# Fadi987/PL-BERT

Measured on AMD Instinct MI355X. Metric: phoneme-tokens/sec, higher is better.
Workload: dtype bf16; 1 GPU; PL-BERT masked-phoneme training step (fwd+loss+bwd+allreduce+AdamW), ALBERT hidden 768 / 12 shared layers / FFN 2048 / 12 heads, seq_len 512, batch 32 per GPU; global_batch=32, seq_len=512, parallelism=dp1

## Files before the change

### plbert_amd/csrc/engine.cpp

```cpp
#include <dlfcn.h>
#include <hip/hip_runtime.h>
#include <math.h>
#include <stdarg.h>
#include <stdio.h>
#include <stdlib.h>
#include <string.h>

#include <array>
#include <map>
#include <new>
#include <string>

#include "../../include/plbert.h"
#include "plbert_kernels.h"

static thread_local char g_err[512] = "";
static int fail(const char* fmt, ...) {
  va_list ap;
  va_start(ap, fmt);
  vsnprintf(g_err, sizeof(g_err), fmt, ap);
  va_end(ap);
  return 1;
}
extern "C" const char* plb_last_error(void) { return g_err; }
// ... 126 lines not shown
  void access(int st, const void* p, size_t bytes, bool wr, const char* what) {
    if (!p || !bytes) return;
    const uintptr_t a = (uintptr_t)p, b = a + bytes;
    vc[st][st] += 1;
    for (const Acc& x : log) {
      if (x.st == st || !(wr || x.wr) || x.b <= a || b <= x.a) continue;
      ++checks;
      if (x.tick > vc[st][x.st]) {
        if (!violations++) {
          char m[384];
          snprintf(m, sizeof(m), "%s of '%s' on the %s stream is not ordered after the %s of '%s' on the %s stream", wr ? "write" : "read",
                   what, name(st), x.wr ? "write" : "read", x.what, name(x.st));
          first = m;
        }
      }
    }
    log.push_back(Acc{what, a, b, st, vc[st][st], wr});
  }
  void new_call() { log.clear(); waits = 0; }
};

}

struct PlbEngine {
  PlbConfig c;
  int64_t poff[PLB_NPARAM], psize[PLB_NPARAM], ptotal, ptrain;
  int E, H, I, L, NH, V, P, NP, NT;
  int64_t Tcap;
  int64_t NMcap;
  int64_t o_wbf, o_wqkvT, o_wdT, o_w1T, o_w2T, o_wpT, o_winT;
  int64_t o_e, o_x, o_qkv, o_ctx, o_pre1, o_a, o_u, o_g, o_pre2;
  int64_t o_lse, o_delta, o_mean1, o_rstd1, o_mean2, o_rstd2;
  int64_t o_dqkv, o_dpre1, o_du, o_dpre2;
  int64_t o_dy0, o_dy1, o_da, o_dctx, o_de;
  int64_t o_hm, o_logm, o_dlog, o_dhm, o_rows, o_tgt, o_w, o_lrows;
  int64_t o_slab, o_part1, o_part2, o_parte, o_scratch, o_dxe, o_ducol, o_slab2, o_scratch2, o_qkvcol = 0;
  int qkvcol_rows = 0;
  int64_t slab2_floats;
  int NTp = 0;
  int64_t o_bt = 0, o_wtT = 0, o_tdl = 0, o_tlrows = 0, o_tscr = 0, o_tgrad = 0, o_tloss = 0;
  int64_t o_tpmax = 0, o_tpsum = 0, o_ttl = 0, o_tlse = 0, o_tw = 0, o_ttgt = 0, o_tcolp = 0;
  bool tok_pad_zeroed = false;
  bool tok_grads_live = false;
  hipStream_t side = nullptr;
  hipEvent_t ev_fork = nullptr, ev_join = nullptr;
  int64_t slab_floats;
  int64_t ws_bytes;
  int ln_blocks, emb_blocks;
  int part_rows = 0;
  int part_rows_used = 0;
  int ln_fuse = 3;
  int64_t o_lnx = 0, o_lnerr = 0, lnx_bytes = 0;
  unsigned int* host_err = nullptr;
  unsigned int* host_err_dev = nullptr;
  bool gelu_dstash_on = true;
  bool u_is_derivative = false;
  bool fp8_on = false, fp8_ready = false, fp8_bwd_ready = false, fp8_wstale = true;
  bool fp8_tn = true;
  bool tn8_call = false;
  int64_t o_x8 = 0, o_a8 = 0, o_g8 = 0, o_c8 = 0, o_dp8 = 0, o_du8 = 0, o_dp18 = 0, o_dq8 = 0;
  int64_t o_wq8 = 0, o_wd8 = 0, o_w18 = 0, o_w28 = 0, o_w2T8 = 0, o_w1T8 = 0, o_wqT8 = 0, o_wdT8 = 0;
  int64_t o_f8amax = 0, o_f8scale = 0, o_f8deq = 0, o_f8stats = 0;
  int f8n = 0;
  bool infer = false;
  int pruned_rows = 0;
  int64_t last_app_rows[2] = {0, 0};
  int64_t last_exec_rows[2] = {0, 0};
// ... 127 lines not shown
  if (tr) {
    e->o_wqkvT = cv.take(rup(H, 128) * 3 * H * 2);
    e->o_wdT = cv.take(rup(H, 128) * H * 2);
    e->o_w1T = cv.take(rup(H, 128) * I * 2);
    e->o_w2T = cv.take(rup(I, 128) * H * 2);
    e->o_wpT = cv.take(rup(H, 128) * 256 * 2);
    e->o_winT = cv.take(rup(E, 128) * H * 2);
  }
  e->o_e = cv.take(Tp * E * 2);
  e->o_x = cv.take((tr ? L + 1 : 2) * Tp * H * 2);
  e->o_qkv = cv.take(Ls * Tp * 3 * H * 2);
  e->o_ctx = cv.take(Ls * Tp * H * 2);
  e->o_pre1 = cv.take(Ls * Tp * H * 2);
  e->o_a = cv.take(Ls * Tp * H * 2);
  e->o_u = cv.take(Ls * Tp * I * 2);
  e->o_g = cv.take(Ls * Tp * I * 2);
  e->o_pre2 = cv.take(Ls * Tp * H * 2);
  const int64_t stat = (int64_t)c.max_batch * e->NH * c.max_seq * 4;
  e->o_lse = cv.take(Ls * stat);
  e->o_mean1 = cv.take(Ls * Tp * 4); e->o_rstd1 = cv.take(Ls * Tp * 4);
  e->o_mean2 = cv.take(Ls * Tp * 4); e->o_rstd2 = cv.take(Ls * Tp * 4);
  e->lnx_bytes = (Tp / 128) * 16 * 128 * 2 * 8;
  e->o_lnx = cv.take(e->lnx_bytes);
  e->o_lnerr = cv.take(256);
  if (tr) {
    e->o_delta = cv.take(stat);
    e->o_dqkv = cv.take(L * Tp * 3 * H * 2);
    e->o_dpre1 = cv.take(L * Tp * H * 2);
    e->o_du = cv.take(L * Tp * I * 2);
    e->o_dpre2 = cv.take(L * Tp * H * 2);
    e->o_dy0 = cv.take(Tp * H * 2); e->o_dy1 = cv.take(Tp * H * 2);
    e->o_da = cv.take(Tp * H * 2); e->o_dctx = cv.take(Tp * H * 2);
    e->o_de = cv.take(Tp * E * 2);
  }
  const int64_t NM = e->NMcap;
  e->o_hm = cv.take(NM * H * 2);
  e->o_logm = cv.take(NM * 256 * 4);
  e->o_dlog = cv.take(NM * 256 * 2);
  e->o_rows = cv.take(NM * 4); e->o_tgt = cv.take(NM * 4); e->o_w = cv.take(NM * 4); e->o_lrows = cv.take(NM * 4);
  if (tr) {
    e->o_dhm = cv.take(NM * H * 2);
    int64_t slab = 0;
    {
      const int64_t Mtot = L * Tp;
      const int ntp = (int)rup(e->NT, 256);
      const int shapes[7][2] = {{(int)(3 * H), (int)H}, {(int)H, (int)H}, {(int)I, (int)H}, {(int)H, (int)I}, {(int)H, (int)E}, {e->NP, (int)H}, {ntp, (int)H}};
      for (int i = 0; i < (e->NT ? 7 : 6); ++i) {
        int rps;
        const int64_t mt = i < 4 ? Mtot : Tp;
        const int s = tn_splits(mt, shapes[i][0], shapes[i][1], &rps);
        const int64_t f = (int64_t)s * shapes[i][0] * shapes[i][1];
        if (f > slab) slab = f;
      }
    }
    e->slab_floats = slab;
    e->o_slab = cv.take(slab * 4);
    e->o_part1 = cv.take(L * e->part_rows * 3 * H * 4);
    e->o_part2 = cv.take(L * e->part_rows * 3 * H * 4);
    e->o_parte = cv.take((int64_t)e->emb_blocks * 2 * E * 4);
    e->o_dxe = cv.take(Tp * E * 4);
    e->o_ducol = cv.take(L * (2 * Tp / 128) * I * 4);
    e->qkvcol_rows = c.max_batch * ((c.max_seq + 127) / 128) * 4;
    e->o_qkvcol = cv.take((int64_t)L * e->qkvcol_rows * 3 * H * 4);
    e->o_scratch = cv.take(512 * (3 * H > I ? 3 * H : I) * 4);
    e->o_scratch2 = cv.take(512 * (3 * H > I ? 3 * H : I) * 4);
    {
// ... 418 lines not shown
}
static int gemm_ln_bwd(PlbEngine* e, PlbGemmNT* g, const F8Op* f8, bool fused, const LnSlot& ln, int nblocks, bf16_t* dx, int T,
                       int Tzero, uint8_t* dx8, const F8Site& q, hipStream_t s) {
  if (fused) {
    g->C = dx; g->aux = ln.pre; g->ldaux = e->H; g->colpart = ln.partials;
    ln_fields(e, g, ln.gamma, nullptr, ln.mean, ln.rstd);
    if (dx8) f8_out(g, dx8, e->H, q, 1);
    TRY(gemm_nt_ln_any(g, 6, f8, s));
    return 0;
  }
  TRY(gemm_nt_any(g, 0, f8, s));
  return ln_bwd(e, ln, nblocks, g->C, dx, T, Tzero, dx8, q, s);
}

static bool tn8_ok(const PlbEngine* e, int64_t Mtot);
static bool f8_call(const PlbEngine* e, int64_t Tp, bool train) {
  return e->fp8_on && e->fp8_ready && (!train || e->fp8_bwd_ready) && fp8_shapes_ok(e, Tp);
}
struct Prune { const int32_t* rows; int n; int Mc; };
static int g_prune_last = -1;
extern "C" void plb_set_prune_last(int on) { g_prune_last = on < 0 ? -1 : (on ? 1 : 0); }
static bool prune_enabled() {
  static const bool v = [] { const char* e = getenv("PLBERT_PRUNE_LAST"); return !(e && !strcmp(e, "0")); }();
  return g_prune_last < 0 ? v : g_prune_last != 0;
}
static int last_application_fwd_pruned(PlbEngine* e, const Prune* pr, bool stash, bool calib, bool tn8, const Slots& sl,
                                       const bf16_t* ctx_att, hipStream_t s) {
  const int H = e->H, I = e->I, L = e->L, Mc = pr->Mc, n = pr->n;
  const F8Site sA(e, F8_A, L - 1), sG(e, F8_G, L - 1), sC(e, F8_C, L - 1);
  bf16_t* ctxc = stash ? sl.ctx : sl.pre1;
  bf16_t* xc = stash ? e->at<bf16_t>(e->o_da) : sl.a;
  bf16_t* pre1c = stash ? sl.pre1 : sl.ctx;
  bf16_t* ac = stash ? sl.a : sl.pre1;
  TRY(plb_launch_gather_rows(ctx_att, H, pr->rows, n, Mc, H, ctxc, H, s));
  TRY(plb_launch_gather_rows(sl.x, H, pr->rows, n, Mc, H, xc, H, s));
  PlbGemmNT g = nt_desc(ctxc, e->wbf(PLB_DENSE_W), Mc, H, H);
  g.bias = e->par(PLB_DENSE_B); g.res = xc; g.ldr = H; g.C = pre1c; g.ldc = H;
  const LnSlot ln1 = {e->par(PLB_LN1_W), e->par(PLB_LN1_B), pre1c, sl.mean1, sl.rstd1, nullptr};
  if (gemm_ln_fwd(e, &g, nullptr, false, ln1, ac, Mc, nullptr, F8Site(), s)) return 1;
  if (calib) TRY(plb_launch_amax(ac, 1, (size_t)n, H, H, sA.amax, s));
  g = nt_desc(ac, e->wbf(PLB_FFN_W), Mc, I, H);
  g.bias = e->par(PLB_FFN_B); g.C = sl.u; g.ldc = I; g.C2 = sl.g; g.ldc2 = I;
  TRY(plb_launch_gemm_nt(&g, 1, 0, s));
  if (calib) TRY(plb_launch_amax(sl.g, 1, (size_t)n, I, I, sG.amax, s));
  g = nt_desc(sl.g, e->wbf(PLB_FFNO_W), Mc, H, I);
  g.bias = e->par(PLB_FFNO_B); g.res = ac; g.ldr = H; g.C = sl.pre2; g.ldc = H;
  if (gemm_ln_fwd(e, &g, nullptr, false, ln2_slot(e, sl), e->at<bf16_t>(e->o_hm), Mc, nullptr, F8Site(), s)) return 1;
  if (tn8) {
    const void* src[3] = {ctxc, ac, sl.g}; const int fl[3] = {1, 1, 1};
    const size_t nel[3] = {(size_t)Mc * H, (size_t)Mc * H, (size_t)Mc * I};
    const float* sc[3] = {sC.scale, sA.scale, sG.scale};
    uint8_t* dst[3] = {sl.c8, sl.a8, sl.g8};
    float* am[3] = {sC.amax, sA.amax, sG.amax};
    TRY(plb_launch_quantize_multi(3, src, fl, nel, sc, dst, am, s));
  }
  return 0;
}

static int run_encoder(PlbEngine* e, const int64_t* ids, const int32_t* lengths, int B, int S, const Rows& rw, bool stash,
                       bf16_t** xout, hipStream_t s, const Prune* pr = nullptr) {
  const int E = e->E, H = e->H, I = e->I, L = e->L;
  const int T = rw.T;
  const int64_t Tp = rw.Tp;
  const bool f8 = f8_call(e, Tp, stash);
  const bool calib = e->fp8_on && !f8;
  if (e->fp8_on && e->fp8_wstale) TRY(fp8_quantize_weights(e, s));
  PlbEmbed em;
  memset(&em, 0, sizeof(em));
// ... 439 lines not shown

static int last_application_bwd_pruned(PlbEngine* e, const Bwd& c, const Slots& sl, const Prune* pr) {
  const int H = e->H, I = e->I, L = e->L, Mc = pr->Mc, n = pr->n;
  hipStream_t s = c.s;
  const F8Site sDP(e, F8_DP, L - 1), sDU(e, F8_DU, L - 1), sDP1(e, F8_DP1, L - 1);
  bf16_t* const dac = e->at<bf16_t>(e->o_da);
  bf16_t* const dctxc = e->at<bf16_t>(e->o_dy0);
  bf16_t* const dctx = e->at<bf16_t>(e->o_dctx);
  if (ln_bwd(e, ln2_slot(e, sl), c.prows, e->at<bf16_t>(e->o_dhm), sl.dpre2, Mc, Mc, nullptr, F8Site(), s)) return 1;
  if (c.calib) TRY(plb_launch_amax(sl.dpre2, 1, (size_t)n, H, H, sDP.amax, s));
  PlbGemmNT g = nt_desc(sl.dpre2, e->at<bf16_t>(e->o_w2T), Mc, I, H);
  g.aux = sl.u; g.ldaux = I; g.C = sl.du; g.ldc = I;
  TRY(plb_launch_gemm_nt(&g, 2, 0, s));
  if (c.calib) TRY(plb_launch_amax(sl.du, 1, (size_t)n, I, I, sDU.amax, s));
  if (c.du_rows > 0) {
    TRY(plb_launch_colsum(sl.du, 1, (size_t)Mc, I, I, sl.ducol, I, 0, e->at<float>(e->o_scratch), 16, s));
    if (c.du_rows > 1) HIPTRY(hipMemsetAsync(sl.ducol + I, 0, (size_t)(c.du_rows - 1) * I * 4, s));
  }
  g = nt_desc(sl.du, e->at<bf16_t>(e->o_w1T), Mc, H, I);
  g.res = sl.dpre2; g.ldr = H; g.C = dac; g.ldc = H;
  if (gemm_ln_bwd(e, &g, nullptr, false, ln1_slot(e, sl), c.prows, sl.dpre1, Mc, Mc, nullptr, F8Site(), s)) return 1;
  if (c.calib) TRY(plb_launch_amax(sl.dpre1, 1, (size_t)n, H, H, sDP1.amax, s));
  if (e->tn8_call) {
    const void* src[3] = {sl.dpre2, sl.du, sl.dpre1}; const int fl[3] = {3, 3, 3};
    const size_t nel[3] = {(size_t)Mc * H, (size_t)Mc * I, (size_t)Mc * H};
    const float* sc[3] = {sDP.scale, sDU.scale, sDP1.scale};
    uint8_t* dst[3] = {sl.dp8, sl.du8, sl.dp18};
    float* am[3] = {sDP.amax, sDU.amax, sDP1.amax};
    TRY(plb_launch_quantize_multi(3, src, fl, nel, sc, dst, am, s));
  }
  g = nt_desc(sl.dpre1, e->at<bf16_t>(e->o_wdT), Mc, H, H);
  g.C = dctxc; g.ldc = H;
  TRY(plb_launch_gemm_nt(&g, 0, 0, s));
  HIPTRY(hipMemsetAsync(dctx, 0, (size_t)c.Tp * H * 2, s));
  TRY(plb_launch_scatter_rows(dctxc, H, pr->rows, n, H, dctx, H, s));
  HIPTRY(hipMemsetAsync(dac, 0, (size_t)c.Tp * H * 2, s));
  TRY(plb_launch_scatter_rows(sl.dpre1, H, pr->rows, n, H, dac, H, s));
  return 0;
}

static int attention_bwd_dx(PlbEngine* e, const Bwd& c, int l, const Slots& sl, bf16_t* ctx, const bf16_t* res,
                            bf16_t* dx) {
  const int H = e->H, T = c.T;
  hipStream_t s = c.s;
  const F8Site sDQ(e, F8_DQ, l);
  PlbAttn at;
  memset(&at, 0, sizeof(at));
  at.qkv = sl.qkv; at.ldqkv = 3 * H; at.lengths = c.lengths; at.B = c.B; at.S = c.S; at.NH = e->NH; at.H = H; at.scale = 0.125f;
  at.row_start = c.row_start;
  at.ctx = ctx; at.ldctx = H; at.lse = sl.lse;
  at.dctx = e->at<bf16_t>(e->o_dctx); at.lddctx = H; at.delta = e->at<float>(e->o_delta); at.dqkv = sl.dqkv; at.lddqkv = 3 * H;
  at.colpart = sl.qkvcol; at.colpart_accumulate = 0;
  if (c.f8) {
    at.dqkv8 = sl.dq8; at.lddqkv8 = 3 * H; at.dqkv_scale = sDQ.scale; at.dqkv_amax = sDQ.amax;
    if (e->tn8_call) at.dqkv = nullptr;
  }
  TRY(plb_launch_attn_bwd(&at, s));
  if (c.Tp > T) {
    if (at.dqkv) HIPTRY(hipMemsetAsync(sl.dqkv + (int64_t)T * 3 * H, 0, (size_t)(c.Tp - T) * 3 * H * 2, s));
    if (c.f8) HIPTRY(hipMemsetAsync(sl.dq8 + (int64_t)T * 3 * H, 0, (size_t)(c.Tp - T) * 3 * H, s));
  }
  if (c.calib) TRY(plb_launch_amax(sl.dqkv, 1, (size_t)T, 3 * H, 3 * H, sDQ.amax, s));
  PlbGemmNT g = nt_desc(sl.dqkv, e->at<bf16_t>(e->o_wqkvT), c.Tp, H, 3 * H);
  g.res = res; g.ldr = H; g.C = dx; g.ldc = H;
  const F8Op ox = f8_op(sl.dq8, sDQ, F8Weight(e, F8W_QKVT), 1);
  if (l == 0) {
    TRY(gemm_nt_any(&g, 0, c.f8 ? &ox : nullptr, s));
    return 0;
  }
  const Slots below = slots(e, c.Tp, c.B, c.S, l - 1, true, c.prows, c.du_rows);
// ... 537 lines not shown
```

### plbert_amd/csrc/gemm.hip

```cpp
#include "common.h"
#include "plbert_kernels.h"
#include "gemm_epilogue.h"

namespace {

constexpr int BM = 128, BN = 128, BK = 64;

DEVI int nt_lds_off(int row, int chunk) { return row * BK + ((chunk ^ ((row >> 1) & 7)) << 3); }

template <int ACT, bool OUTF32>
__global__ __launch_bounds__(256) void gemm_nt_kernel(PlbGemmNT p) {
  __shared__ __attribute__((aligned(16))) bf16_t smem[2][2][BM * BK];
  const int tid = threadIdx.x, lane = tid & 63, wave = tid >> 6;
  const int wr = wave >> 1, wc = wave & 1;
  const int nbn = (p.N + BN - 1) / BN;
  const int nwg = gridDim.x;
  const int logical = xcd_remap(blockIdx.x, nwg);
  const int bm = logical / nbn, bn = logical % nbn;

  const int uw = __builtin_amdgcn_readfirstlane(wave);
  const int drow = lane >> 3, dch = lane & 7;
  const bf16_t* gA = p.A + (size_t)(bm * BM + uw * 32 + drow) * p.lda;
  const bf16_t* gB = p.B + (size_t)(bn * BN + uw * 32 + drow) * p.ldb;
  const size_t sa = (size_t)8 * p.lda, sb = (size_t)8 * p.ldb;
  int sch[4];
#pragma unroll
  for (int i = 0; i < 4; ++i) sch[i] = (dch ^ ((4 * i + (lane >> 4)) & 7)) * 8;
  typedef __attribute__((address_space(1))) const void* gptr_t;
  typedef __attribute__((address_space(3))) void* lptr_t;
#define NT_STAGE(st, kt)                                                                              \
  do {                                                                                                \
    _Pragma("unroll") for (int i = 0; i < 4; ++i) {                                                   \
      __builtin_amdgcn_global_load_lds((gptr_t)(gA + i * sa + (size_t)(kt) * BK + sch[i]),            \
                                       (lptr_t)&smem[st][0][(uw * 32 + i * 8) * BK], 16, 0, 0);       \
      __builtin_amdgcn_global_load_lds((gptr_t)(gB + i * sb + (size_t)(kt) * BK + sch[i]),            \
                                       (lptr_t)&smem[st][1][(uw * 32 + i * 8) * BK], 16, 0, 0);       \
    }                                                                                                 \
  } while (0)
#define NT_LANDED() asm volatile("s_waitcnt vmcnt(0)" ::: "memory")

  f32x4 acc[4][4];
#pragma unroll
  for (int i = 0; i < 4; ++i)
#pragma unroll
    for (int j = 0; j < 4; ++j) acc[i][j] = f32x4{0.f, 0.f, 0.f, 0.f};

  const int frow = lane & 15, fq = lane >> 4;
  const int fsw = (frow >> 1) & 7;
  const int offA = (wr * 64 + frow) * BK, offB = (wc * 64 + frow) * BK;
#define NT_COMPUTE(st)                                                                                   \
  do {                                                                                                   \
    const bf16_t* sA = smem[st][0];                                                                      \
    const bf16_t* sB = smem[st][1];                                                                      \
    _Pragma("unroll") for (int kk = 0; kk < 2; ++kk) {                                                   \
      const int ch = ((kk * 4 + fq) ^ fsw) << 3;                                                         \
      bf16x8 af[4], bfr[4];                                                                              \
      _Pragma("unroll") for (int i = 0; i < 4; ++i) {                                                    \
        af[i] = *(const bf16x8*)&sA[offA + i * 16 * BK + ch];                                            \
        bfr[i] = *(const bf16x8*)&sB[offB + i * 16 * BK + ch];                                           \
      }                                                                                                  \
      _Pragma("unroll") for (int mi = 0; mi < 4; ++mi)                                                   \
        _Pragma("unroll") for (int ni = 0; ni < 4; ++ni)                                                 \
          acc[mi][ni] = __builtin_amdgcn_mfma_f32_16x16x32_bf16(bfr[ni], af[mi], acc[mi][ni], 0, 0, 0);  \
    }                                                                                                    \
  } while (0)

  const int nk = p.K / BK;
  NT_STAGE(0, 0);
  NT_LANDED();
  __syncthreads();
  for (int kt = 0; kt < nk; ++kt) {
    const int cur = kt & 1;
    if (kt + 1 < nk) NT_STAGE(cur ^ 1, kt + 1);
    NT_COMPUTE(cur);
    NT_LANDED();
    __syncthreads();
  }
#undef NT_STAGE
#undef NT_LANDED
#undef NT_COMPUTE

#pragma unroll
  for (int mi = 0; mi < 4; ++mi) {
    const int m = bm * BM + wr * 64 + mi * 16 + frow;
#pragma unroll
    for (int ni = 0; ni < 4; ++ni)
      nt_epilogue<ACT, OUTF32>(p, acc[mi][ni], m, bn * BN + wc * 64 + ni * 16 + fq * 4);
  }
}

DEVI int tn_unit(int t) { return (t & 3) | (((t >> 3) & 1) << 2) | (((t >> 2) & 1) << 3) | (t & 48); }
DEVI int tn_lds_off(int t, int col) {
  int s = col >> 4;
  return s * 1024 + (((tn_unit(t) + s) & 63) << 4) + (col & 15);
}

__global__ __launch_bounds__(256) void gemm_tn_kernel(PlbGemmTN p) {
  __shared__ __attribute__((aligned(16))) bf16_t smem[2][2][64 * 128];
  const int tid = threadIdx.x, lane = tid & 63, wave = tid >> 6;
  const int wn = wave >> 1, wk = wave & 1;
  const int nbk = (p.K + 127) / 128;
  const int bn = blockIdx.x / nbk, bk = blockIdx.x % nbk;
  const int split = blockIdx.y;
  const int t_begin = split * p.rows_per_split;
  int t_end = t_begin + p.rows_per_split;
  if (t_end > p.Mtot) t_end = p.Mtot;
  const int nt = (t_end - t_begin) / 64;

  const int lc = tid & 15, lr = tid >> 4;
  const int colA = bn * 128 + lc * 8, colB = bk * 128 + lc * 8;
  const bool okA = colA < p.Ncols, okB = colB < p.K;
  uint4 ra[4], rb[4];
  auto load_tile = [&](int it) {
    const size_t t0 = (size_t)t_begin + (size_t)it * 64 + lr;
#pragma unroll
    for (int i = 0; i < 4; ++i) {
      ra[i] = okA ? *(const uint4*)(p.A + (t0 + 16 * i) * p.lda + colA) : make_uint4(0, 0, 0, 0);
      rb[i] = okB ? *(const uint4*)(p.B + (t0 + 16 * i) * p.ldb + colB) : make_uint4(0, 0, 0, 0);
    }
  };
// ... 38 lines not shown
        bfr[i] = bf16x8{b0[0], b0[1], b0[2], b0[3], b1[0], b1[1], b1[2], b1[3]};
      }
#pragma unroll
      for (int ni = 0; ni < 4; ++ni)
#pragma unroll
        for (int ki = 0; ki < 4; ++ki)
          acc[ni][ki] = __builtin_amdgcn_mfma_f32_16x16x32_bf16(bfr[ki], af[ni], acc[ni][ki], 0, 0, 0);
    }
    if (it + 1 < nt) store_tile(cur ^ 1);
    __syncthreads();
  }

  float* out = p.slab + (size_t)split * p.N * p.K;
#pragma unroll
  for (int ni = 0; ni < 4; ++ni) {
    const int n = bn * 128 + wn * 64 + ni * 16 + li;
    if (n >= p.N) continue;
#pragma unroll
    for (int ki = 0; ki < 4; ++ki) {
      const int k0 = bk * 128 + wk * 64 + ki * 16 + 4 * g;
      if (k0 >= p.K) continue;
      f32x4 v = acc[ni][ki];
      *(float4*)(out + (size_t)n * p.K + k0) = make_float4(v[0], v[1], v[2], v[3]);
    }
  }
}

}

static int g_nt_tile = 0;
extern "C" void plb_set_gemm_nt_tile(int tile) { g_nt_tile = tile; }
extern "C" int plb_launch_gemm_nt_big(const PlbGemmNT* p, int tile, int act, int out_f32, hipStream_t stream);

static int pick_tile(const PlbGemmNT* p) {
  const bool ok256 = p->M % 256 == 0 && p->N % 256 == 0, ok384 = p->M % 128 == 0 && p->N % 384 == 0;
  const bool ok1256 = p->M % 128 == 0 && p->N % 256 == 0;
  if (g_nt_tile == 128) return 128;
  if (g_nt_tile == 256) return ok256 ? 256 : 128;
  if (g_nt_tile == 384) return ok384 ? 384 : (ok256 ? 256 : 128);
  if (g_nt_tile == 1256) return ok1256 ? 1256 : 128;
  if ((long)p->M * p->N < 256L * 256 * 64) return 128;
  double e256 = 0, e384 = 0, e1256 = 0;
  if (ok256) { const long t = (long)(p->M / 256) * (p->N / 256); e256 = (double)t / (double)(((t + 255) / 256) * 256); }
  if (ok384) { const long t = (long)(p->M / 128) * (p->N / 384); e384 = 0.95 * (double)t / (double)(((t + 255) / 256) * 256); }
  if (ok1256) { const long t = (long)(p->M / 128) * (p->N / 256); e1256 = 0.85 * (double)t / (double)(((t + 255) / 256) * 256); }
  if (e256 == 0 && e384 == 0 && e1256 == 0) return 128;
  if (e1256 > e256 && e1256 > e384) return 1256;
  return e384 > e256 ? 384 : 256;
}

extern "C" int plb_gemm_nt_colpart_rows(int M, int N, int K) {
  PlbGemmNT q;
  q.M = M; q.N = N; q.K = K;
  const int tile = pick_tile(&q);
  return tile == 256 ? 2 * (M / 256) : (tile == 384 || tile == 1256) ? 2 * (M / 128) : 0;
}

extern "C" int plb_launch_gemm_nt(const PlbGemmNT* p, int act, int out_f32, hipStream_t stream) {
  if (p->M % BM || p->K % BK || p->N % 4 || p->M <= 0 || p->N <= 0 || p->K <= 0) return 1;
  const int nbn = (p->N + BN - 1) / BN;
  dim3 grid((p->M / BM) * nbn), block(256);
  const int cls = out_f32 ? PLB_K_GEMM_NT_F32 : act == 1 ? PLB_K_GEMM_NT_GELU : act == 2 ? PLB_K_GEMM_NT_GELUBWD : PLB_K_GEMM_NT;
  const int tile = pick_tile(p);
  if (p->colpart && tile == 128) return 1;
  const double mnk = (double)p->M * p->N * p->K;
  const double algo_bytes = 2.0 * ((double)p->M * p->K + (double)p->N * p->K) +
                            (double)p->M * p->N * (out_f32 ? 4 : act == 1 ? 4 : 2) +
                            (p->res ? 2.0 * p->M * p->N : 0.0) + (act == 2 ? 2.0 * p->M * p->N : 0.0);
  if (tile != 128) {
    const int tokb = plb_prof_begin(cls, stream, 2.0 * mnk, algo_bytes);
    const int rc = plb_launch_gemm_nt_big(p, tile, act, out_f32, stream);
    plb_prof_end(tokb, stream);
    return rc;
  }
  const int tok = plb_prof_begin(out_f32 ? PLB_K_GEMM_NT_F32 : PLB_K_GEMM_NT_SMALL, stream, 2.0 * mnk, algo_bytes);
  if (out_f32) {
    if (act != 0) return 1;
    hipLaunchKernelGGL((gemm_nt_kernel<0, true>), grid, block, 0, stream, *p);
  } else if (act == 0) {
    hipLaunchKernelGGL((gemm_nt_kernel<0, false>), grid, block, 0, stream, *p);
  } else if (act == 1) {
    hipLaunchKernelGGL((gemm_nt_kernel<1, false>), grid, block, 0, stream, *p);
  } else if (act == 2) {
    hipLaunchKernelGGL((gemm_nt_kernel<2, false>), grid, block, 0, stream, *p);
  } else {
    return 1;
  }
  plb_prof_end(tok, stream);
  return hipGetLastError() == hipSuccess ? 0 : 2;
}

extern "C" int plb_launch_gemm_tn(const PlbGemmTN* p, hipStream_t stream) {
  if (p->Mtot % 64 || p->rows_per_split % 64 || p->K % 4 || p->N <= 0 || p->splits <= 0) return 1;
  if ((long)p->splits * p->rows_per_split < p->Mtot) return 1;
  dim3 grid(((p->N + 127) / 128) * ((p->K + 127) / 128), p->splits), block(256);
  const int tok = plb_prof_begin(PLB_K_GEMM_TN, stream, 2.0 * p->Mtot * (double)p->N * p->K,
                                 2.0 * p->Mtot * ((double)p->N + p->K) + 4.0 * p->splits * (double)p->N * p->K);
  hipLaunchKernelGGL(gemm_tn_kernel, grid, block, 0, stream, *p);
  plb_prof_end(tok, stream);
  return hipGetLastError() == hipSuccess ? 0 : 2;
}
```

### plbert_amd/csrc/plbert_kernels.h

```cpp
#pragma once
#include <hip/hip_runtime.h>
#include <stdint.h>

typedef uint16_t bf16_t;

extern "C" {

enum PlbKernelClass {
  PLB_K_GEMM_NT = 0, PLB_K_GEMM_NT_GELU, PLB_K_GEMM_NT_GELUBWD, PLB_K_GEMM_NT_F32, PLB_K_GEMM_TN,
  PLB_K_ATTN_FWD, PLB_K_ATTN_BWD_DQ, PLB_K_ATTN_BWD_DKV, PLB_K_LN_FWD, PLB_K_LN_BWD, PLB_K_EMBED_FWD,
  PLB_K_EMBED_BWD, PLB_K_COLSUM, PLB_K_REDUCE, PLB_K_ROWS, PLB_K_CE, PLB_K_ADAMW, PLB_K_CAST, PLB_K_TOKEN_CE, PLB_K_GEMM_NT_CE, PLB_K_GEMM_NT_SMALL, PLB_K_FP8, PLB_K_ATTN_BWD,
  PLB_K_GEMM_NT_FP8, PLB_K_GEMM_NT_GELU_FP8, PLB_K_GEMM_NT_GELUBWD_FP8,
  PLB_K_GEMM_NT_LNFWD, PLB_K_GEMM_NT_LNBWD,
  PLB_K_GEMM_NT_LNFWD_FP8, PLB_K_GEMM_NT_LNBWD_FP8, PLB_K_GEMM_TN_FP8,
  PLB_K_NCLASS
};
int plb_prof_begin(int cls, hipStream_t s, double flops, double bytes);
void plb_prof_end(int tok, hipStream_t s);

typedef struct {
  const bf16_t* A; int lda;
  const bf16_t* B; int ldb;
  int M, N, K;
  int Mstore;
// ... 94 lines not shown
int plb_launch_copy_cols(const float* scratch, int nsplit, int N, int col0, int Nout, float* out, hipStream_t stream);

int plb_launch_pooler(const float* hidden, int B, int S, int H, const float* W, const float* bias, float* pooled,
                      hipStream_t stream);

typedef struct {
  const bf16_t* qkv; int ldqkv;
  const int32_t* lengths;
  int B, S, NH, H;
  float scale;
  bf16_t* ctx; int ldctx;
  float* lse;
  const bf16_t* dctx; int lddctx;
  float* delta;
  bf16_t* dqkv; int lddqkv;
  float* colpart;
  int colpart_accumulate;
  uint8_t* ctx8; int ldctx8; const float* ctx_scale; float* ctx_amax;
  uint8_t* dqkv8; int lddqkv8; const float* dqkv_scale; float* dqkv_amax;
  const int32_t* qoff; const bf16_t* q; int ldq; int nq_total; bf16_t* dq; int lddq; uint8_t* dq8; int lddq8;
  const int32_t* row_start;
} PlbAttn;
int plb_launch_attn_fwd(const PlbAttn* p, hipStream_t stream);
int plb_launch_attn_bwd(const PlbAttn* p, hipStream_t stream);
int plb_launch_attn_bwd_fused(const PlbAttn* p, hipStream_t stream);
void plb_debug_skip_piece(int index);
void plb_debug_ln_fault(int mode, int launches);
void plb_set_attn_bwd_fused(int on);

int plb_launch_gather_rows(const bf16_t* src, int lds_, const int32_t* rows, int n, int npad, int H, bf16_t* dst,
                           int ldd, hipStream_t stream);
int plb_launch_scatter_rows(const bf16_t* src, int lds_, const int32_t* rows, int n, int H, bf16_t* dst, int ldd,
                            hipStream_t stream);
int plb_launch_ce_prepare(const int32_t* offsets, const int32_t* flat, const int64_t* labels, int B, int S,
                          int32_t* rows, int32_t* tgt, float* w, hipStream_t stream);
int plb_launch_ce_prepare_packed(const int32_t* offsets, const int32_t* flat, const int64_t* labels, int B, int S,
                                 const int32_t* row_start, int32_t* rows, int32_t* tgt, float* w, hipStream_t stream);
int plb_launch_unpack_rows(const void* src, int src_is_bf16, int lds_, const int32_t* row_start, const int32_t* lengths,
                           int B, int S, int C, float* dst, hipStream_t stream);
int plb_launch_ce_fwd_bwd(const float* logits, int ldl, int V, const int32_t* tgt, const float* w, int n, int npad,
                          float* loss_rows, bf16_t* dlogits, int ldd, hipStream_t stream);
int plb_launch_sum_rows(const float* x, int n, float* out, hipStream_t stream);
int plb_launch_token_ce_combine(const float* pmax, const float* psum, int ntiles, const float* tlogit,
                                const int32_t* lengths, int B, int S, int rows, float* lse, float* w, float* loss_rows,
                                hipStream_t stream);
int plb_launch_add_scalar(float* out, const float* a, const float* b, hipStream_t stream);

typedef struct {
  const int64_t* labels; const int32_t* lengths;
  int B, S;
  uint64_t seed; uint32_t step;
  float word_pred_prob, mask_prob, replace_prob;
  int mask_id, sep_id;
  int64_t* masked; int32_t *counts, *idx_padded, *offsets, *flat;
} PlbMask;
int plb_launch_mask(const PlbMask* p, hipStream_t stream);

typedef struct {
  const int64_t* ids; const int32_t *sample_off, *word_off, *word_begin, *word_len; const int8_t* action;
  const int64_t* repl; const int64_t* word_token; int64_t sep_token; const int32_t* crop_start;
  int B, S, mask_id;
  int64_t *labels, *masked, *tokens; int32_t *lengths_out, *counts, *idx_padded, *offsets, *flat;
} PlbApplyMask;
int plb_launch_apply_mask(const PlbApplyMask* p, hipStream_t stream);

int plb_launch_adamw(float* p, const float* g, float* m, float* v, bf16_t* p_bf16, size_t n, double lr, double beta1,
// ... 12 lines not shown
```

### plbert_amd/csrc/rowops.hip

```cpp
#include "common.h"
#include "plbert_kernels.h"

namespace {

__device__ __forceinline__ bool packed_locate(const int32_t* row_start, const int32_t* lengths, int B, int S, int r, int* b_out,
                                              int* s_out) {
  int lo = 0, hi = B;
  while (hi - lo > 1) {
    const int mid = (lo + hi) >> 1;
    if (row_start[mid] <= r) lo = mid; else hi = mid;
  }
  int len = lengths[lo];
  len = len < 1 ? 1 : (len > S ? S : len);
  *b_out = lo; *s_out = r - row_start[lo];
  return *s_out < len;
}

template <bool BWD>
__global__ __launch_bounds__(256) void embed_kernel(PlbEmbed p) {
  const int lane = threadIdx.x & 63, wave = threadIdx.x >> 6;
  const int E = p.E;
  const int c = lane * 4;
  const bool act = c < E;
  float4 g4 = make_float4(0, 0, 0, 0), b4 = g4, ty = g4;
// ... 665 lines not shown
    int k = g;
    for (; k + 24 < nsplit; k += 32) {
      s0 += px[(size_t)k * N]; s1 += px[(size_t)(k + 8) * N]; s2 += px[(size_t)(k + 16) * N]; s3 += px[(size_t)(k + 24) * N];
    }
    for (; k < nsplit; k += 8) s0 += px[(size_t)k * N];
  }
  red[g][c] = (s0 + s1) + (s2 + s3);
  __syncthreads();
  if (g == 0 && j < Nout) {
    const float t = ((red[0][c] + red[1][c]) + (red[2][c] + red[3][c])) + ((red[4][c] + red[5][c]) + (red[6][c] + red[7][c]));
    out[j] = accumulate ? out[j] + t : t;
  }
}

__global__ void gather_rows_kernel(const bf16_t* src, int lds_, const int32_t* rows, int n, int npad, int H,
                                   bf16_t* dst, int ldd) {
  const int r = blockIdx.x;
  const int chunks = H / 8;
  const bool live = r < n;
  const size_t srow = live ? (size_t)rows[r] : 0;
  for (int c = threadIdx.x; c < chunks; c += blockDim.x) {
    uint4 v = live ? *(const uint4*)(src + srow * lds_ + c * 8) : make_uint4(0, 0, 0, 0);
    *(uint4*)(dst + (size_t)r * ldd + c * 8) = v;
  }
}
__global__ void scatter_rows_kernel(const bf16_t* src, int lds_, const int32_t* rows, int n, int H, bf16_t* dst,
                                    int ldd) {
  const int r = blockIdx.x;
  if (r >= n) return;
  const size_t drow = (size_t)rows[r];
  for (int c = threadIdx.x; c < H / 8; c += blockDim.x)
    *(uint4*)(dst + drow * ldd + c * 8) = *(const uint4*)(src + (size_t)r * lds_ + c * 8);
}
__global__ void ce_prepare_kernel(const int32_t* offsets, const int32_t* flat, const int64_t* labels, int B, int S,
                                  const int32_t* row_start, int32_t* rows, int32_t* tgt, float* w) {
  __shared__ int cnt[4];
  int c = 0;
  for (int b = threadIdx.x; b < B; b += blockDim.x) c += offsets[b + 1] > offsets[b];
  c = (int)wave_sum((float)c);
  if ((threadIdx.x & 63) == 0) cnt[threadIdx.x >> 6] = c;
  __syncthreads();
  const int count = cnt[0] + cnt[1] + cnt[2] + cnt[3];
  const int b = blockIdx.x;
  const int j0 = offsets[b], j1 = offsets[b + 1];
  const float wb = (j1 > j0) ? 1.0f / ((float)(j1 - j0) * (float)count) : 0.f;
  for (int j = j0 + threadIdx.x; j < j1; j += blockDim.x) {
    const int idx = flat[j];
    rows[j] = row_start ? row_start[b] + idx : b * S + idx;
    tgt[j] = (int32_t)labels[(size_t)b * S + idx];
    w[j] = wb;
  }
}
template <typename T>
__global__ __launch_bounds__(256) void unpack_rows_kernel(const T* src, int lds_, const int32_t* row_start, const int32_t* lengths,
                                                          int S, int C, float* dst) {
  const int b = blockIdx.x / S, s = blockIdx.x - b * S;
  int len = lengths[b];
  len = len < 1 ? 1 : (len > S ? S : len);
  float* d = dst + (size_t)blockIdx.x * C;
  if (s >= len) {
    for (int c = threadIdx.x; c < C; c += 256) d[c] = 0.f;
    return;
  }
  const T* r = src + (size_t)(row_start[b] + s) * lds_;
  for (int c = threadIdx.x; c < C; c += 256) {
    if constexpr (sizeof(T) == 2) d[c] = bf2f(r[c]); else d[c] = r[c];
// ... 370 lines not shown
                                 int accumulate, float* scratch, int nsplit, hipStream_t stream) {
  if (N % 8 || ld % 8 || nsplit <= 0 || Nout > N) return 1;
  ProfScope ps(PLB_K_COLSUM, stream, 0, (double)R * N * (is_bf16 ? 2 : 4));
  dim3 grid((N + 255) / 256, nsplit);
  if (is_bf16) hipLaunchKernelGGL((colsum_kernel<true>), grid, dim3(256), 0, stream, X, R, N, ld, scratch, nsplit);
  else hipLaunchKernelGGL((colsum_kernel<false>), grid, dim3(256), 0, stream, X, R, N, ld, scratch, nsplit);
  if (hipGetLastError() != hipSuccess) return 2;
  hipLaunchKernelGGL(reduce_cols_kernel, dim3((unsigned)((Nout + 31) / 32)), dim3(256), 0, stream, scratch, nsplit, N,
                     Nout, out, accumulate, 0);
  return LAUNCH_OK();
}
extern "C" int plb_launch_copy_cols(const float* scratch, int nsplit, int N, int col0, int Nout, float* out,
                                    hipStream_t stream) {
  if (nsplit <= 0 || col0 < 0 || col0 + Nout > N) return 1;
  hipLaunchKernelGGL(reduce_cols_kernel, dim3((unsigned)((Nout + 31) / 32)), dim3(256), 0, stream, scratch, nsplit, N,
                     Nout, out, 0, col0);
  return LAUNCH_OK();
}
extern "C" int plb_launch_gather_rows(const bf16_t* src, int lds_, const int32_t* rows, int n, int npad, int H,
                                      bf16_t* dst, int ldd, hipStream_t stream) {
  if (H % 8 || npad <= 0) return 1;
  ProfScope ps(PLB_K_ROWS, stream, 0, 4.0 * (double)npad * H);
  hipLaunchKernelGGL(gather_rows_kernel, dim3(npad), dim3(128), 0, stream, src, lds_, rows, n, npad, H, dst, ldd);
  return LAUNCH_OK();
}
extern "C" int plb_launch_scatter_rows(const bf16_t* src, int lds_, const int32_t* rows, int n, int H, bf16_t* dst,
                                       int ldd, hipStream_t stream) {
  if (H % 8) return 1;
  if (n <= 0) return 0;
  hipLaunchKernelGGL(scatter_rows_kernel
, dim3(n), dim3(128), 0, stream, src, lds_, rows, n, H, dst, ldd);
  return LAUNCH_OK();
}
extern "C" int plb_launch_ce_prepare(const int32_t* offsets, const int32_t* flat, const int64_t* labels, int B, int S,
                                     int32_t* rows, int32_t* tgt, float* w, hipStream_t stream) {
  hipLaunchKernelGGL(ce_prepare_kernel, dim3(B), dim3(256), 0, stream, offsets, flat, labels, B, S, nullptr, rows, tgt, w);
  return LAUNCH_OK();
}
extern "C" int plb_launch_ce_prepare_packed(const int32_t* offsets, const int32_t* flat, const int64_t* labels, int B, int S,
                                            const int32_t* row_start, int32_t* rows, int32_t* tgt, float* w,
                                            hipStream_t stream) {
  if (!row_start || B < 1 || S < 1) return 1;
  hipLaunchKernelGGL(ce_prepare_kernel, dim3(B), dim3(256), 0, stream, offsets, flat, labels, B, S, row_start, rows, tgt, w);
  return LAUNCH_OK();
}
extern "C" int plb_launch_unpack_rows(const void* src, int src_is_bf16, int lds_, const int32_t* row_start,
                                      const int32_t* lengths, int B, int S, int C, float* dst, hipStream_t stream) {
  if (!src || !row_start || !lengths || !dst || B < 1 || S < 1 || C < 1 || lds_ < C) return 1;
  ProfScope ps(PLB_K_CAST, stream, 0, (double)B * S * C * 6.0);
  if (src_is_bf16)
    hipLaunchKernelGGL(unpack_rows_kernel<bf16_t>, dim3((unsigned)(B * S)), dim3(256), 0, stream, (const bf16_t*)src, lds_,
                       row_start, lengths, S, C, dst);
  else
    hipLaunchKernelGGL(unpack_rows_kernel<float>, dim3((unsigned)(B * S)), dim3(256), 0, stream, (const float*)src, lds_,
                       row_start, lengths, S, C, dst);
  return LAUNCH_OK();
}
extern "C" int plb_launch_ce_fwd_bwd(const float* logits, int ldl, int V, const int32_t* tgt, const float* w, int n,
                                     int npad, float* loss_rows, bf16_t* dlogits, int ldd, hipStream_t stream) {
  if (V > 256 || ldd > 256 || ldd % 4 || npad <= 0) return 1;
  ProfScope ps(PLB_K_CE, stream, 0, (double)npad * (4.0 * V + 2.0 * ldd));
  hipLaunchKernelGGL(ce_kernel, dim3((npad + 3) / 4), dim3(256), 0, stream, logits, ldl, V, tgt, w, n, npad, loss_rows,
                     dlogits, ldd);
  return LAUNCH_OK();
}
extern "C" int plb_launch_token_ce_combine(const float* pmax, const float* psum, int ntiles, const float* tlogit,
// ... 121 lines not shown
```

Baseline: 1.771 million tokens/s.

## Add 64x64 small-GEMM tile path and fuse pruned-layer gather/scatter kernels

Templates the small NT GEMM kernel on tile size and picks a 64x64 tile when a 128x128 tiling would launch too few workgroups to fill the GPU. This aims to raise occupancy for small GEMMs such as the pruned last layer. Separately, it merges the two gather-rows launches into one 2-D launch that also records an inverse row map. The two memset+scatter pairs in the pruned backward become one kernel that writes zeros or scattered rows for every token. The inverse map is never cleared, so it relies on the rows[j]==t check to reject stale entries.

```diff
diff --git a/plbert_amd/csrc/engine.cpp b/plbert_amd/csrc/engine.cpp
--- a/plbert_amd/csrc/engine.cpp
+++ b/plbert_amd/csrc/engine.cpp
@@ -182,7 +182,7 @@
   int64_t o_e, o_x, o_qkv, o_ctx, o_pre1, o_a, o_u, o_g, o_pre2;
   int64_t o_lse, o_delta, o_mean1, o_rstd1, o_mean2, o_rstd2;
   int64_t o_dqkv, o_dpre1, o_du, o_dpre2;
-  int64_t o_dy0, o_dy1, o_da, o_dctx, o_de;
+  int64_t o_dy0, o_dy1, o_da, o_dctx, o_de, o_rowinv;
   int64_t o_hm, o_logm, o_dlog, o_dhm, o_rows, o_tgt, o_w, o_lrows;
   int64_t o_slab, o_part1, o_part2, o_parte, o_scratch, o_dxe, o_ducol, o_slab2, o_scratch2, o_qkvcol = 0;
   int qkvcol_rows = 0;
@@ -376,6 +376,7 @@
     e->o_dy0 = cv.take(Tp * H * 2); e->o_dy1 = cv.take(Tp * H * 2);
     e->o_da = cv.take(Tp * H * 2); e->o_dctx = cv.take(Tp * H * 2);
     e->o_de = cv.take(Tp * E * 2);
+    e->o_rowinv = cv.take(Tp * 4);
   }
   const int64_t NM = e->NMcap;
   e->o_hm = cv.take(NM * H * 2);
@@ -860,8 +861,7 @@
   bf16_t* xc = stash ? e->at<bf16_t>(e->o_da) : sl.a;
   bf16_t* pre1c = stash ? sl.pre1 : sl.ctx;
   bf16_t* ac = stash ? sl.a : sl.pre1;
-  TRY(plb_launch_gather_rows(ctx_att, H, pr->rows, n, Mc, H, ctxc, H, s));
-  TRY(plb_launch_gather_rows(sl.x, H, pr->rows, n, Mc, H, xc, H, s));
+  TRY(plb_launch_gather_rows2(ctx_att, sl.x, H, pr->rows, n, Mc, H, ctxc, xc, H, stash ? e->at<int32_t>(e->o_rowinv) : nullptr, s));
   PlbGemmNT g = nt_desc(ctxc, e->wbf(PLB_DENSE_W), Mc, H, H);
   g.bias = e->par(PLB_DENSE_B); g.res = xc; g.ldr = H; g.C = pre1c; g.ldc = H;
   const LnSlot ln1 = {e->par(PLB_LN1_W), e->par(PLB_LN1_B), pre1c, sl.mean1, sl.rstd1, nullptr};
@@ -1367,10 +1367,7 @@
   g = nt_desc(sl.dpre1, e->at<bf16_t>(e->o_wdT), Mc, H, H);
   g.C = dctxc; g.ldc = H;
   TRY(plb_launch_gemm_nt(&g, 0, 0, s));
-  HIPTRY(hipMemsetAsync(dctx, 0, (size_t)c.Tp * H * 2, s));
-  TRY(plb_launch_scatter_rows(dctxc, H, pr->rows, n, H, dctx, H, s));
-  HIPTRY(hipMemsetAsync(dac, 0, (size_t)c.Tp * H * 2, s));
-  TRY(plb_launch_scatter_rows(sl.dpre1, H, pr->rows, n, H, dac, H, s));
+  TRY(plb_launch_scatter_rows_zero2(dctxc, sl.dpre1, H, pr->rows, e->at<int32_t>(e->o_rowinv), n, (int)c.Tp, H, dctx, dac, H, s));
   return 0;
 }
 
diff --git a/plbert_amd/csrc/gemm.hip b/plbert_amd/csrc/gemm.hip
--- a/plbert_amd/csrc/gemm.hip
+++ b/plbert_amd/csrc/gemm.hip
@@ -4,24 +4,33 @@
 
 namespace {
 
-constexpr int BM = 128, BN = 128, BK = 64;
+constexpr int BM = 128, BK = 64;
 
 DEVI int nt_lds_off(int row, int chunk) { return row * BK + ((chunk ^ ((row >> 1) & 7)) << 3); }
 
-template <int ACT, bool OUTF32>
+template <int TILE> struct NtTile {
+  static_assert(TILE == 128 || TILE == 64, "square tiles of 128 or 64");
+  static constexpr int TM = TILE, TN = TILE;
+  static constexpr int MI = TM / 32, NI = TN / 32;
+  static constexpr int IA = TM / 32, IB = TN / 32;
+};
+
+template <int ACT, bool OUTF32, int TILE>
 __global__ __launch_bounds__(256) void gemm_nt_kernel(PlbGemmNT p) {
-  __shared__ __attribute__((aligned(16))) bf16_t smem[2][2][BM * BK];
+  typedef NtTile<TILE> T;
+  constexpr int TM = T::TM, TN = T::TN, MI = T::MI, NI = T::NI, IA = T::IA, IB = T::IB;
+  __shared__ __attribute__((aligned(16))) bf16_t smem[2][(TM + TN) * BK];
   const int tid = threadIdx.x, lane = tid & 63, wave = tid >> 6;
   const int wr = wave >> 1, wc = wave & 1;
-  const int nbn = (p.N + BN - 1) / BN;
+  const int nbn = (p.N + TN - 1) / TN;
   const int nwg = gridDim.x;
   const int logical = xcd_remap(blockIdx.x, nwg);
   const int bm = logical / nbn, bn = logical % nbn;
 
   const int uw = __builtin_amdgcn_readfirstlane(wave);
   const int drow = lane >> 3, dch = lane & 7;
-  const bf16_t* gA = p.A + (size_t)(bm * BM + uw * 32 + drow) * p.lda;
-  const bf16_t* gB = p.B + (size_t)(bn * BN + uw * 32 + drow) * p.ldb;
+  const bf16_t* gA = p.A + (size_t)(bm * TM + uw * 8 * IA + drow) * p.lda;
+  const bf16_t* gB = p.B + (size_t)(bn * TN + uw * 8 * IB + drow) * p.ldb;
   const size_t sa = (size_t)8 * p.lda, sb = (size_t)8 * p.ldb;
   int sch[4];
 #pragma unroll
@@ -31,36 +40,35 @@
 #define NT_STAGE(st, kt)                                                                              \
   do {                                                                                                \
     _Pragma("unroll") for (int i = 0; i < 4; ++i) {                                                   \
-      __builtin_amdgcn_global_load_lds((gptr_t)(gA + i * sa + (size_t)(kt) * BK + sch[i]),            \
-                                       (lptr_t)&smem[st][0][(uw * 32 + i * 8) * BK], 16, 0, 0);       \
-      __builtin_amdgcn_global_load_lds((gptr_t)(gB + i * sb + (size_t)(kt) * BK + sch[i]),            \
-                                       (lptr_t)&smem[st][1][(uw * 32 + i * 8) * BK], 16, 0, 0);       \
+      if (i < IA)                                                                                     \
+        __builtin_amdgcn_global_load_lds((gptr_t)(gA + i * sa + (size_t)(kt) * BK + sch[i]),          \
+                                         (lptr_t)&smem[st][(uw * 8 * IA + i * 8) * BK], 16, 0, 0);    \
+      if (i < IB)                                                                                     \
+        __builtin_amdgcn_global_load_lds((gptr_t)(gB + i * sb + (size_t)(kt) * BK + sch[i]),          \
+                                         (lptr_t)&smem[st][(TM + uw * 8 * IB + i * 8) * BK], 16, 0, 0); \
     }                                                                                                 \
   } while (0)
 #define NT_LANDED() asm volatile("s_waitcnt vmcnt(0)" ::: "memory")
 
-  f32x4 acc[4][4];
-#pragma unroll
-  for (int i = 0; i < 4; ++i)
-#pragma unroll
-    for (int j = 0; j < 4; ++j) acc[i][j] = f32x4{0.f, 0.f, 0.f, 0.f};
+  f32x4 acc[MI][NI];
+#pragma unroll
+  for (int i = 0; i < MI; ++i)
+#pragma unroll
+    for (int j = 0; j < NI; ++j) acc[i][j] = f32x4{0.f, 0.f, 0.f, 0.f};
 
   const int frow = lane & 15, fq = lane >> 4;
   const int fsw = (frow >> 1) & 7;
-  const int offA = (wr * 64 + frow) * BK, offB = (wc * 64 + frow) * BK;
+  const int offA = (wr * 16 * MI + frow) * BK, offB = (TM + wc * 16 * NI + frow) * BK;
 #define NT_COMPUTE(st)                                                                                   \
   do {                                                                                                   \
-    const bf16_t* sA = smem[st][0];                                                                      \
-    const bf16_t* sB = smem[st][1];                                                                      \
+    const bf16_t* sm = smem[st];                                                                         \
     _Pragma("unroll") for (int kk = 0; kk < 2; ++kk) {                                                   \
       const int ch = ((kk * 4 + fq) ^ fsw) << 3;                                                         \
-      bf16x8 af[4], bfr[4];                                                                              \
-      _Pragma("unroll") for (int i = 0; i < 4; ++i) {                                                    \
-        af[i] = *(const bf16x8*)&sA[offA + i * 16 * BK + ch];                                            \
-        bfr[i] = *(const bf16x8*)&sB[offB + i * 16 * BK + ch];                                           \
-      }                                                                                                  \
-      _Pragma("unroll") for (int mi = 0; mi < 4; ++mi)                                                   \
-        _Pragma("unroll") for (int ni = 0; ni < 4; ++ni)                                                 \
+      bf16x8 af[MI], bfr[NI];                                                                            \
+      _Pragma("unroll") for (int i = 0; i < MI; ++i) af[i] = *(const bf16x8*)&sm[offA + i * 16 * BK + ch];   \
+      _Pragma("unroll") for (int i = 0; i < NI; ++i) bfr[i] = *(const bf16x8*)&sm[offB + i * 16 * BK + ch];  \
+      _Pragma("unroll") for (int mi = 0; mi < MI; ++mi)                                                  \
+        _Pragma("unroll") for (int ni = 0; ni < NI; ++ni)                                                \
           acc[mi][ni] = __builtin_amdgcn_mfma_f32_16x16x32_bf16(bfr[ni], af[mi], acc[mi][ni], 0, 0, 0);  \
     }                                                                                                    \
   } while (0)
@@ -81,11 +89,11 @@
 #undef NT_COMPUTE
 
 #pragma unroll
-  for (int mi = 0; mi < 4; ++mi) {
-    const int m = bm * BM + wr * 64 + mi * 16 + frow;
-#pragma unroll
-    for (int ni = 0; ni < 4; ++ni)
-      nt_epilogue<ACT, OUTF32>(p, acc[mi][ni], m, bn * BN + wc * 64 + ni * 16 + fq * 4);
+  for (int mi = 0; mi < MI; ++mi) {
+    const int m = bm * TM + wr * 16 * MI + mi * 16 + frow;
+#pragma unroll
+    for (int ni = 0; ni < NI; ++ni)
+      nt_epilogue<ACT, OUTF32>(p, acc[mi][ni], m, bn * TN + wc * 16 * NI + ni * 16 + fq * 4);
   }
 }
 
@@ -190,22 +198,28 @@
 extern "C" void plb_set_gemm_nt_tile(int tile) { g_nt_tile = tile; }
 extern "C" int plb_launch_gemm_nt_big(const PlbGemmNT* p, int tile, int act, int out_f32, hipStream_t stream);
 
+constexpr long NT_WG_FILL = 512;
+static int pick_small_tile(const PlbGemmNT* p) {
+  return (long)(p->M / 128) * ((p->N + 127) / 128) >= NT_WG_FILL ? 128 : 64;
+}
+
 static int pick_tile(const PlbGemmNT* p) {
   const bool ok256 = p->M % 256 == 0 && p->N % 256 == 0, ok384 = p->M % 128 == 0 && p->N % 384 == 0;
   const bool ok1256 = p->M % 128 == 0 && p->N % 256 == 0;
-  if (g_nt_tile == 128) return 128;
+  if (g_nt_tile == 128 || g_nt_tile == 64) return g_nt_tile;
   if (g_nt_tile == 256) return ok256 ? 256 : 128;
   if (g_nt_tile == 384) return ok384 ? 384 : (ok256 ? 256 : 128);
   if (g_nt_tile == 1256) return ok1256 ? 1256 : 128;
-  if ((long)p->M * p->N < 256L * 256 * 64) return 128;
+  if ((long)p->M * p->N < 256L * 256 * 64) return pick_small_tile(p);
   double e256 = 0, e384 = 0, e1256 = 0;
   if (ok256) { const long t = (long)(p->M / 256) * (p->N / 256); e256 = (double)t / (double)(((t + 255) / 256) * 256); }
   if (ok384) { const long t = (long)(p->M / 128) * (p->N / 384); e384 = 0.95 * (double)t / (double)(((t + 255) / 256) * 256); }
   if (ok1256) { const long t = (long)(p->M / 128) * (p->N / 256); e1256 = 0.85 * (double)t / (double)(((t + 255) / 256) * 256); }
-  if (e256 == 0 && e384 == 0 && e1256 == 0) return 128;
+  if (e256 == 0 && e384 == 0 && e1256 == 0) return pick_small_tile(p);
   if (e1256 > e256 && e1256 > e384) return 1256;
   return e384 > e256 ? 384 : 256;
 }
+static bool small_tile(int tile) { return tile == 128 || tile == 64; }
 
 extern "C" int plb_gemm_nt_colpart_rows(int M, int N, int K) {
   PlbGemmNT q;
@@ -214,36 +228,41 @@
   return tile == 256 ? 2 * (M / 256) : (tile == 384 || tile == 1256) ? 2 * (M / 128) : 0;
 }
 
+template <int TILE>
+static int launch_nt_small(const PlbGemmNT* p, int act, int out_f32, hipStream_t stream) {
+  typedef NtTile<TILE> T;
+  dim3 grid((p->M / T::TM) * ((p->N + T::TN - 1) / T::TN)), block(256);
+  if (out_f32) {
+    hipLaunchKernelGGL((gemm_nt_kernel<0, true, TILE>), grid, block, 0, stream, *p);
+  } else if (act == 0) {
+    hipLaunchKernelGGL((gemm_nt_kernel<0, false, TILE>), grid, block, 0, stream, *p);
+  } else if (act == 1) {
+    hipLaunchKernelGGL((gemm_nt_kernel<1, false, TILE>), grid, block, 0, stream, *p);
+  } else {
+    hipLaunchKernelGGL((gemm_nt_kernel<2, false, TILE>), grid, block, 0, stream, *p);
+  }
+  return 0;
+}
+
 extern "C" int plb_launch_gemm_nt(const PlbGemmNT* p, int act, int out_f32, hipStream_t stream) {
   if (p->M % BM || p->K % BK || p->N % 4 || p->M <= 0 || p->N <= 0 || p->K <= 0) return 1;
-  const int nbn = (p->N + BN - 1) / BN;
-  dim3 grid((p->M / BM) * nbn), block(256);
   const int cls = out_f32 ? PLB_K_GEMM_NT_F32 : act == 1 ? PLB_K_GEMM_NT_GELU : act == 2 ? PLB_K_GEMM_NT_GELUBWD : PLB_K_GEMM_NT;
   const int tile = pick_tile(p);
-  if (p->colpart && tile == 128) return 1;
+  if (p->colpart && small_tile(tile)) return 1;
   const double mnk = (double)p->M * p->N * p->K;
   const double algo_bytes = 2.0 * ((double)p->M * p->K + (double)p->N * p->K) +
                             (double)p->M * p->N * (out_f32 ? 4 : act == 1 ? 4 : 2) +
                             (p->res ? 2.0 * p->M * p->N : 0.0) + (act == 2 ? 2.0 * p->M * p->N : 0.0);
-  if (tile != 128) {
+  if (!small_tile(tile)) {
     const int tokb = plb_prof_begin(cls, stream, 2.0 * mnk, algo_bytes);
     const int rc = plb_launch_gemm_nt_big(p, tile, act, out_f32, stream);
     plb_prof_end(tokb, stream);
     return rc;
   }
+  if (act < 0 || act > 2 || (out_f32 && act != 0)) return 1;
   const int tok = plb_prof_begin(out_f32 ? PLB_K_GEMM_NT_F32 : PLB_K_GEMM_NT_SMALL, stream, 2.0 * mnk, algo_bytes);
-  if (out_f32) {
-    if (act != 0) return 1;
-    hipLaunchKernelGGL((gemm_nt_kernel<0, true>), grid, block, 0, stream, *p);
-  } else if (act == 0) {
-    hipLaunchKernelGGL((gemm_nt_kernel<0, false>), grid, block, 0, stream, *p);
-  } else if (act == 1) {
-    hipLaunchKernelGGL((gemm_nt_kernel<1, false>), grid, block, 0, stream, *p);
-  } else if (act == 2) {
-    hipLaunchKernelGGL((gemm_nt_kernel<2, false>), grid, block, 0, stream, *p);
-  } else {
-    return 1;
-  }
+  if (tile == 64) launch_nt_small<64>(p, act, out_f32, stream);
+  else launch_nt_small<128>(p, act, out_f32, stream);
   plb_prof_end(tok, stream);
   return hipGetLastError() == hipSuccess ? 0 : 2;
 }
diff --git a/plbert_amd/csrc/plbert_kernels.h b/plbert_amd/csrc/plbert_kernels.h
--- a/plbert_amd/csrc/plbert_kernels.h
+++ b/plbert_amd/csrc/plbert_kernels.h
@@ -150,6 +150,10 @@
                            int ldd, hipStream_t stream);
 int plb_launch_scatter_rows(const bf16_t* src, int lds_, const int32_t* rows, int n, int H, bf16_t* dst, int ldd,
                             hipStream_t stream);
+int plb_launch_gather_rows2(const bf16_t* src0, const bf16_t* src1, int lds_, const int32_t* rows, int n, int npad, int H,
+                            bf16_t* dst0, bf16_t* dst1, int ldd, int32_t* inv, hipStream_t stream);
+int plb_launch_scatter_rows_zero2(const bf16_t* src0, const bf16_t* src1, int lds_, const int32_t* rows, const int32_t* inv,
+                                  int n, int T, int H, bf16_t* dst0, bf16_t* dst1, int ldd, hipStream_t stream);
 int plb_launch_ce_prepare(const int32_t* offsets, const int32_t* flat, const int64_t* labels, int B, int S,
                           int32_t* rows, int32_t* tgt, float* w, hipStream_t stream);
 int plb_launch_ce_prepare_packed(const int32_t* offsets, const int32_t* flat, const int64_t* labels, int B, int S,
diff --git a/plbert_amd/csrc/rowops.hip b/plbert_amd/csrc/rowops.hip
--- a/plbert_amd/csrc/rowops.hip
+++ b/plbert_amd/csrc/rowops.hip
@@ -721,6 +721,31 @@
   for (int c = threadIdx.x; c < H / 8; c += blockDim.x)
     *(uint4*)(dst + drow * ldd + c * 8) = *(const uint4*)(src + (size_t)r * lds_ + c * 8);
 }
+__global__ void gather_rows2_kernel(const bf16_t* src0, const bf16_t* src1, int lds_, const int32_t* rows, int n, int H,
+                                    bf16_t* dst0, bf16_t* dst1, int ldd, int32_t* inv) {
+  const int r = blockIdx.x;
+  const bf16_t* src = blockIdx.y ? src1 : src0;
+  bf16_t* dst = blockIdx.y ? dst1 : dst0;
+  const bool live = r < n;
+  const size_t srow = live ? (size_t)rows[r] : 0;
+  if (live && inv && blockIdx.y == 0 && threadIdx.x == 0) inv[srow] = r;
+  for (int c = threadIdx.x; c < H / 8; c += blockDim.x) {
+    uint4 v = live ? *(const uint4*)(src + srow * lds_ + c * 8) : make_uint4(0, 0, 0, 0);
+    *(uint4*)(dst + (size_t)r * ldd + c * 8) = v;
+  }
+}
+__global__ void scatter_rows_zero2_kernel(const bf16_t* src0, const bf16_t* src1, int lds_, const int32_t* rows,
+                                          const int32_t* inv, int n, int H, bf16_t* dst0, bf16_t* dst1, int ldd) {
+  const int t = blockIdx.x;
+  const bf16_t* src = blockIdx.y ? src1 : src0;
+  bf16_t* dst = blockIdx.y ? dst1 : dst0;
+  const int j = inv[t];
+  const bool live = j >= 0 && j < n && rows[j] == t;
+  for (int c = threadIdx.x; c < H / 8; c += blockDim.x) {
+    uint4 v = live ? *(const uint4*)(src + (size_t)j * lds_ + c * 8) : make_uint4(0, 0, 0, 0);
+    *(uint4*)(dst + (size_t)t * ldd + c * 8) = v;
+  }
+}
 __global__ void ce_prepare_kernel(const int32_t* offsets, const int32_t* flat, const int64_t* labels, int B, int S,
                                   const int32_t* row_start, int32_t* rows, int32_t* tgt, float* w) {
   __shared__ int cnt[4];
@@ -1157,6 +1182,23 @@
 , dim3(n), dim3(128), 0, stream, src, lds_, rows, n, H, dst, ldd);
   return LAUNCH_OK();
 }
+extern "C" int plb_launch_gather_rows2(const bf16_t* src0, const bf16_t* src1, int lds_, const int32_t* rows, int n, int npad,
+                                       int H, bf16_t* dst0, bf16_t* dst1, int ldd, int32_t* inv, hipStream_t stream) {
+  if (H % 8 || npad <= 0 || n < 0 || n > npad) return 1;
+  ProfScope ps(PLB_K_ROWS, stream, 0, 8.0 * (double)npad * H);
+  hipLaunchKernelGGL(gather_rows2_kernel, dim3(npad, 2), dim3(128), 0, stream, src0, src1, lds_, rows, n, H, dst0, dst1, ldd,
+                     inv);
+  return LAUNCH_OK();
+}
+extern "C" int plb_launch_scatter_rows_zero2(const bf16_t* src0, const bf16_t* src1, int lds_, const int32_t* rows,
+                                             const int32_t* inv, int n, int T, int H, bf16_t* dst0, bf16_t* dst1, int ldd,
+                                             hipStream_t stream) {
+  if (H % 8 || T <= 0 || n < 0 || !inv) return 1;
+  ProfScope ps(PLB_K_ROWS, stream, 0, 4.0 * (double)T * H + 4.0 * (double)n * H);
+  hipLaunchKernelGGL(scatter_rows_zero2_kernel, dim3(T, 2), dim3(128), 0, stream, src0, src1, lds_, rows, inv, n, H, dst0,
+                     dst1, ldd);
+  return LAUNCH_OK();
+}
 extern "C" int plb_launch_ce_prepare(const int32_t* offsets, const int32_t* flat, const int64_t* labels, int B, int S,
                                      int32_t* rows, int32_t* tgt, float* w, hipStream_t stream) {
   hipLaunchKernelGGL(ce_prepare_kernel, dim3(B), dim3(256), 0, stream, offsets, flat, labels, B, S, nullptr, rows, tgt, w);
```

Measured after the change: 1.773 million tokens/s, median of 2. About the same (+0.1%).
